# GaodeRender/triangle-splatting

Measured on AMD Instinct MI355X. Metric: fwd+bwd Mpixels/sec @ 1M triangles, 1920x1080; achieved HBM GB/s, higher is better.
Workload: dtype f32

## Files before the change

### triangle-splatting_amd/csrc/api.hip

```cpp
#pragma GCC visibility push(default)
#include "../../include/ts2d.h"
#ifdef TS2D_LAB
#include "ts2d_lab.h"
#endif
#pragma GCC visibility pop
#include "ts2d_api.h"
#include <atomic>
#include <chrono>
#include <cstdarg>
#include <cstdio>
#include <cstring>
#include <mutex>
#include <string>
#include <vector>

namespace
{
thread_local std::string g_err;

struct ProfRow { std::string name; double ms = 0; int64_t launches = 0; };
struct ProfPending { int row; hipEvent_t a, b; };
std::mutex g_prof_mu;
bool g_prof_on = false;
std::string g_prof_only;
std::vector<ProfRow> g_prof_rows;
std::vector<ProfPending> g_prof_pending;
std::vector<hipEvent_t> g_prof_free;

void prof_drain()
{
    for (auto &p : g_prof_pending)
    {
        float ms = 0;
        if (hipEventSynchronize(p.b) == hipSuccess && hipEventElapsedTime(&ms, p.a, p.b) == hipSuccess)
        {
            g_prof_rows[p.row].ms += ms;
            g_prof_rows[p.row].launches += 1;
        }
        g_prof_free.push_back(p.a);
        g_prof_free.push_back(p.b);
    }
    g_prof_pending.clear();
}

#ifdef TS2D_LAB
bool g_lab_all_quadrants = false;
bool g_lab_kernel_cull = false;
#endif

bool block_masks_in_keys(const ts2d_camera *cam, uint32_t flags)
{
    const int gx = (cam->width + TS_TILE - 1) / TS_TILE, gy = (cam->height + TS_TILE - 1) / TS_TILE;
    return !(flags & TS2D_FLAG_3D) && (int64_t)gx * gy <= TS_BLOCKMASK_MAX_TILES;
}

int validate(const ts2d_camera *cam, const ts2d_geometry *geom, uint32_t flags)
{
    if (!cam || !geom) return ts_fail(TS2D_ERR_INVALID, "null camera/geometry");
    if (cam->width <= 0 || cam->height <= 0) return ts_fail(TS2D_ERR_INVALID, "image size must be positive");
    if (cam->width > 65535 * TS_TILE || cam->height > 65535 * TS_TILE) return ts_fail(TS2D_ERR_INVALID, "image too large");
    if (geom->P < 0) return ts_fail(TS2D_ERR_INVALID, "P must be >= 0");
    if (geom->P > (int)TS_ID_MASK) return ts_fail(TS2D_ERR_CAPACITY, "more than 2^28 - 1 triangles: the instance values keep four bits for the quadrant mask");
    if (geom->C > TS2D_MAX_CHANNELS)
        return ts_fail(TS2D_ERR_INVALID, "feature's num_channels can't be larger than MAX_CHANNELS");
    if (geom->C < 1) return ts_fail(TS2D_ERR_INVALID, "need at least one colour channel");
    if (geom->gamma < 0.0f) return ts_fail(TS2D_ERR_INVALID, "gamma must be larger than 0");
    if (flags & TS2D_FLAG_USE_SHS)
    {
        if (geom->C != 3) return ts_fail(TS2D_ERR_INVALID, "SH mode renders 3 channels");
        if (geom->sh_degree < 0 || geom->sh_degree > 3) return ts_fail(TS2D_ERR_INVALID, "sh_degree must be in 0..3");
        if ((geom->sh_degree + 1) * (geom->sh_degree + 1) > geom->M)
            return ts_fail(TS2D_ERR_INVALID, "shs holds fewer coefficients than sh_degree needs");
        if (geom->P > 0 && !geom->shs) return ts_fail(TS2D_ERR_INVALID, "shs is null");
    }
    else if (geom->P > 0 && !geom->feature) return ts_fail(TS2D_ERR_INVALID, "feature is null");
    if (geom->P > 0 && (!geom->vertex || !geom->opacity)) return ts_fail(TS2D_ERR_INVALID, "vertex/opacity is null");
    if (!cam->viewmatrix || !cam->projmatrix || !cam->campos || !geom->background)
        return ts_fail(TS2D_ERR_INVALID, "camera matrices / background are null");
    return TS2D_OK;
}

PreprocessArgs make_pre(const ts2d_camera *cam, const ts2d_geometry *geom, uint32_t flags)
{
    PreprocessArgs a;
    a.W = cam->width; a.H = cam->height; a.P = geom->P; a.D = geom->sh_degree; a.M = geom->M; a.C = geom->C;
    a.grid_x = (cam->width + TS_TILE - 1) / TS_TILE; a.grid_y = (cam->height + TS_TILE - 1) / TS_TILE;
    a.rich_info = flags & TS2D_FLAG_RICH_INFO; a.use_shs = flags & TS2D_FLAG_USE_SHS;
    a.back_culling = flags & TS2D_FLAG_BACK_CULLING;
    a.tan_fovx = cam->tan_fovx; a.tan_fovy = cam->tan_fovy;
    a.viewmatrix = cam->viewmatrix; a.projmatrix = cam->projmatrix; a.campos = cam->campos;
    a.vertex = geom->vertex; a.shs = geom->shs; a.feature = geom->feature; a.opacity = geom->opacity;
    return a;
}

RenderArgs make_render(const ts2d_camera *cam, const ts2d_geometry *geom, uint32_t flags)
{
    RenderArgs r;
    r.W = cam->width; r.H = cam->height; r.C = geom->C;
    r.grid_x = (cam->width + TS_TILE - 1) / TS_TILE; r.grid_y = (cam->height + TS_TILE - 1) / TS_TILE;
    r.gamma = geom->gamma; r.background_depth = geom->background_depth;
    r.background_depth_dev = geom->background_depth_dev;
    r.background = geom->background;
    r.rich_info = flags & TS2D_FLAG_RICH_INFO;
    r.block_masks = block_masks_in_keys(cam, flags);
#ifdef TS2D_LAB
    if (g_lab_kernel_cull) r.block_masks = false;
#endif
    return r;
}

inline void cpu_relax()
{
#if defined(__x86_64__) || defined(__i386__)
    __builtin_ia32_pause();
#elif defined(__aarch64__)
    asm volatile("yield" ::: "memory");
#endif
}

struct CapacityHint { int dev, variant, W, H; unsigned long long key; double per_triangle; unsigned long long stamp; };
thread_local unsigned long long t_hint_key = 0;
std::atomic<unsigned long long> g_speculative_overflows{0};
std::mutex g_hint_mu;
std::vector<CapacityHint> g_hints;
unsigned long long g_hint_clock = 0;

void record_instance_count(int variant, int W, int H, int P, unsigned long long n)
{
    int dev = 0;
    if (P <= 0 || hipGetDevice(&dev) != hipSuccess) return;
    const double per = (double)n / (double)P;
    std::lock_guard<std::mutex> lk(g_hint_mu);
    CapacityHint *slot = nullptr;
    for (auto &h : g_hints)
        if (h.dev == dev && h.variant == variant && h.W == W && h.H == H && h.key == t_hint_key) slot = &h;
    if (!slot)
    {
        if (g_hints.size() < 32) { g_hints.push_back({dev, variant, W, H, t_hint_key, 0.0, 0}); slot = &g_hints.back(); }
        else
// ... 526 lines not shown
        if (dst_bytes < (size_t)N * 8) return ts_fail(TS2D_ERR_CAPACITY, "dst too small");
        std::vector<uint32_t> tile((size_t)N), vals((size_t)N), depth((size_t)P);
        if (N > 0)
        {
            TS_HIP(hipMemcpyAsync(tile.data(), b.tile, (size_t)N * 4, hipMemcpyDeviceToHost, s));
            TS_HIP(hipMemcpyAsync(vals.data(), b.vals, (size_t)N * 4, hipMemcpyDeviceToHost, s));
            TS_HIP(hipMemcpyAsync(depth.data(), g.depth, (size_t)P * 4, hipMemcpyDeviceToHost, s));
            TS_HIP(hipStreamSynchronize(s));
        }
        uint64_t *o = (uint64_t *)dst;
        const uint32_t keymask = ts_tile_keymask(gx * gy);
        for (int64_t i = 0; i < N; i++) o[i] = ((uint64_t)(tile[i] & keymask) << 32) | depth[vals[i] & TS_ID_MASK];
        return TS2D_OK;
    }
    case 11: src = b.vals; bytes = (size_t)N * 4; break;
    case 12: src = im.ranges; bytes = (size_t)gx * gy * 8; break;
    case 13: src = im.n_contrib; bytes = (size_t)W * H * 4; break;
    case 14: src = im.final_T; bytes = (size_t)W * H * 4; break;
    case 15: src = b.k[(b.passes & 1) ^ 1]; bytes = (size_t)N * 4; break;
    case 16: src = b.v[(b.passes & 1) ^ 1]; bytes = (size_t)N * 4; break;
    case 17:
    {
        uint32_t top_const = 0;
        if (P > 0)
        {
            TS_HIP(hipMemcpyAsync(&top_const, g.top_const, 4, hipMemcpyDeviceToHost, s));
            TS_HIP(hipStreamSynchronize(s));
        }
        src = top_const ? g.sv[0] : g.sv[1];
        bytes = (size_t)P * 4;
        break;
    }
    case 18: src = g.rec; bytes = (size_t)P * TS_REC_FLOATS * 4; break;
    default: return ts_fail(TS2D_ERR_INVALID, "unknown field %d", field);
    }
    if (dst_bytes < bytes) return ts_fail(TS2D_ERR_CAPACITY, "dst too small");
    if (bytes)
    {
        TS_HIP(hipMemcpyAsync(dst, src, bytes, hipMemcpyDeviceToHost, s));
        TS_HIP(hipStreamSynchronize(s));
    }
    return TS2D_OK;
}

void ts2d_lab_force_ticket_passes(int on) { ts_force_ticket_passes(on != 0); }
void ts2d_lab_force_all_quadrants(int on) { g_lab_all_quadrants = on != 0; }
void ts2d_lab_force_kernel_cull(int on) { g_lab_kernel_cull = on != 0; }
void ts2d_lab_force_depth_pass4(int on) { ts_force_depth_pass4(on != 0); }
void ts2d_lab_depth_split(int mode, int bucket_cap) { ts_lab_depth_split(mode, bucket_cap); }
#endif

void ts2d_profile_enable(int on)
{
    std::lock_guard<std::mutex> lk(g_prof_mu);
    g_prof_on = on != 0;
}
void ts2d_profile_only(const char *name)
{
    std::lock_guard<std::mutex> lk(g_prof_mu);
    g_prof_only = name ? name : "";
}
void ts2d_profile_reset(void)
{
    std::lock_guard<std::mutex> lk(g_prof_mu);
    prof_drain();
    g_prof_rows.clear();
}
int ts2d_profile_read(int32_t index, char *name, size_t name_bytes, double *total_ms, int64_t *launches)
{
    std::lock_guard<std::mutex> lk(g_prof_mu);
    prof_drain();
    if (index < 0 || (size_t)index >= g_prof_rows.size()) return TS2D_ERR_INVALID;
    const ProfRow &r = g_prof_rows[index];
    if (name && name_bytes) { strncpy(name, r.name.c_str(), name_bytes - 1); name[name_bytes - 1] = 0; }
    if (total_ms) *total_ms = r.ms;
    if (launches) *launches = r.launches;
    return TS2D_OK;
}
}
```

### triangle-splatting_amd/csrc/render_group.hip

```cpp
#include "ts2d_common.h"
#include "ts2d_wave.h"
#include "ts2d_group.h"
#include "ts2d_support.h"

#ifndef TSG_FWD_WAVES
#define TSG_FWD_WAVES 7
#endif
#ifndef TSG_BWD_WAVES
#define TSG_BWD_WAVES 7
#endif
#ifndef TSG_FWD_CAP
#define TSG_FWD_CAP 64
#endif
#ifndef TSG_BWD_CAP
#define TSG_BWD_CAP 64
#endif
#ifndef TSG_TCAP
#define TSG_TCAP 960
#endif
#ifndef TSG_PART
#define TSG_PART 3
#endif
namespace
{
// ... 73 lines not shown
    BlockCull s;
    entry_geometry(s, r0.x, r0.y, r0.z, r0.w, r1.x, r1.y, OX, OY);
#pragma unroll
    for (int g = 0; g < 4; g++) s.ov[g] = (id_nibble >> (TS_ID_BITS + g)) & 1u;
    return s;
}

__device__ __forceinline__ void write_dummy_row(float *row, int lane)
{
    if (lane < ROW)
    {
        float v = 0.0f;
        if (lane == 0 || lane == 1 || lane == 3 || lane == 4) v = 1000.0f;
        if (lane == 2 || lane == 5) v = 1001.0f;
        if (lane == 6) v = 1.0f;
        if (lane == 18) v = __int_as_float(0x7fffffff);
        row[lane] = v;
    }
}

struct Bary { float p1x, p1y, p2x, p2y, p3x, p3y, a1, a2, a3, mn, ecc; };
__device__ __forceinline__ Bary barycentrics(const float4 &q0, const float4 &q1, float fx, float fy)
{
    Bary b;
    b.p1x = q0.x - fx; b.p1y = q0.y - fy; b.p2x = q0.z - fx; b.p2y = q0.w - fy; b.p3x = q1.x - fx; b.p3y = q1.y - fy;
    b.a1 = (b.p2x * b.p3y - b.p2y * b.p3x) * q1.z;
    b.a2 = (b.p3x * b.p1y - b.p3y * b.p1x) * q1.z;
    b.a3 = 1.0f - b.a1 - b.a2;
    b.mn = fminf(fminf(b.a1, b.a2), b.a3);
    b.ecc = fmaf(-3.0f, b.mn, 1.0f);
    return b;
}
#ifdef TS2D_STATS
__device__ unsigned long long g_stats_group[12];
#define TSG_STAT(i, v) stat_acc[i] += (unsigned long long)(v)
#else
#define TSG_STAT(i, v)
#endif

#if TSG_PART & 1
template <bool RICH, bool GAMMA1, bool CULL>
__global__ void __launch_bounds__(256, TSG_FWD_WAVES) render_fwd_group_kernel(RenderArgs a, const uint2 *__restrict__ ranges,
                                                                const uint32_t *__restrict__ point_list, const uint32_t *__restrict__ keys,
                                                                const float4 *__restrict__ rec,
                                                                float *__restrict__ final_T, uint32_t *__restrict__ n_contrib,
                                                                float *__restrict__ out_feature, float *__restrict__ out_depth,
                                                                float *__restrict__ out_normal, float *__restrict__ contrib_sum,
                                                                float *__restrict__ contrib_max)
{
    __shared__ __attribute__((aligned(16))) float cst_all[4][(NR + 1) * ROW];
    __shared__ __attribute__((aligned(16))) uint32_t list_all[4][4 * NR / 2];
    constexpr int TCAP = TSG_TCAP;
    __shared__ unsigned long long tsum[RICH ? TCAP : 1];
    __shared__ int tmax[RICH ? TCAP : 1];

    const int tile = tile_of_block(blockIdx.x, a.grid_x, a.grid_y);
    if (tile < 0) return;
    const int wave = threadIdx.x >> 6;
    const GroupPixel p = group_pixel(a, tile, wave);
    const int lane = p.lane;
    const float fx = (float)p.lx, fy = (float)p.ly, OX = (float)p.X0, OY = (float)p.Y0;
    const uint2 range = ranges[tile];
    const int len = (int)(range.y - range.x);
    if (RICH) tile_stats_clear<TCAP>(tsum, tmax, len);
    const float g2 = 2.0f * a.gamma;
    float *cst = cst_all[wave] + ROW;
    uint32_t *list = list_all[wave];
    write_dummy_row(cst - ROW, lane);
    const char *lds0 = (const char *)cst_all;
    const uint32_t row0 = table_row0(wave, ROW), dummy = row0 - ROW * 4;
    const int stat_step = window_stat_step(lane);
    FwdPixel P = fwd_pixel(p.inside, len);

#ifdef TS2D_STATS
    unsigned long long stat_acc[12] = {0, 0, 0, 0, 0, 1, 0, 0, 0, 0, 0, 0};
#endif
    uint32_t id = 0;
    int pos = 0, cursor = 0;
    for (;;)
    {
        const unsigned long long alive = ballot(!P.done);
        if (alive == 0) break;
        int nq = 0;
        stream_refill<false, TSG_FWD_CAP, !CULL>(id, pos, nq, point_list + range.x, cursor, len, CULL ? TS_ID_BITS + wave : 16 + 4 * wave, lane,
                                                 keys + range.x);
        if (nq == 0) break;
        const bool valid = lane < nq;
        const int ent = pos;
        const uint32_t tid = CULL ? id : id & TS_ID_MASK;
        float4 r0 = make_float4(0, 0, 0, 0), r1 = r0, r2 = r0, r3 = r0;
        gather_record<RICH>(rec, tid, valid, r0, r1, r2, r3);
        const BlockCull s = entry_blocks<GAMMA1, CULL>(r0, r1, id, g2, OX, OY);
        unsigned long long M[4];
        const unsigned long long any = fwd_block_masks(M, alive, valid, s.ov);
        TSG_STAT(0, __popcll(ballot(valid)));
        if (any == 0) continue;
        TSG_STAT(1, __popcll(M[0]) + __popcll(M[1]) + __popcll(M[2]) + __popcll(M[3]));
        TSG_STAT(6, 1);
        TSG_STAT(7, __popcll(any));
        const Compaction cp = compact_rows(any, lane);
        bool mine = in_pass(cp, false);
        if (mine) publish_row(cst + cp.r * ROW, s, tid, ent, r1, r2, r3);
        for (int h = 0;;)
        {
            const int steps = build_lists(list, M, pass_mask(cp, mine), row0, cp.r, ROW, dummy, lane);
            const u16a *mylist = (const u16a *)list + p.grp * NR;
            TSG_STAT(2, steps);
            TSG_STAT(3, (steps + 7) / 8);
            TSG_STAT(8, __popcll(list_conflicts(list, dummy, lane)));
            TSG_STAT(9, 1);
            TSG_STAT(10, h > 0 ? 1 : 0);

            for (int t0 = 0; t0 < steps; t0 += 8)
            {
                float c[8];
                const uint4 packed = *(const uint4 *)(mylist + t0);
#pragma unroll
                for (int st = 0; st < 8; st++)
                {
                    c[st] = 0.0f;
                    if (t0 + st < steps)
                    {
                        const float *row = window_row(lds0, packed, st);
                        const float4 q0 = *(const float4 *)(row), q1 = *(const float4 *)(row + 4);
                        const Bary b = barycentrics(q0, q1, fx, fy);
                        const float4 q2 = *(const float4 *)(row + 8);
                        float4 q3 = make_float4(0, 0, 0, 0);
                        float vd3 = 0.0f;
                        int jpos;
                        if (RICH)
                        {
                            q3 = *(const float4 *)(row + 12);
                            const float4 q4 = *(const float4 *)(row + 16);
                            vd3 = q4.x;
                            jpos = __float_as_int(q4.z);
                        }
                        else jpos = __float_as_int(row[18]);
                        const float pw = GAMMA1 ? b.ecc * b.ecc : pow_nonneg(b.ecc, g2);
                        const float alpha = fminf(0.99f, q1.w * __builtin_amdgcn_exp2f(pw * -0.7213475204444817f));
                        const bool hit = !P.done && ecc_in_range(b.ecc) && alpha >= 1.0f / 255.0f;
                        TSG_STAT(4, __popcll(ballot(hit)));
                        const float d = q3.z * b.a1 + q3.w * b.a2 + vd3 * b.a3;
                        const float contrib = fwd_blend<RICH>(P, hit, alpha, q2.x, q2.y, q2.z, q2.w, q3.x, q3.y, d, jpos);
                        if (RICH) c[st] = contrib;
                    }
                }
                if (RICH) window_stats<TCAP>(c, lane, stat_step, lds0, mylist, t0, 18, tsum, tmax, point_list + range.x, contrib_sum, contrib_max);
            }
            if (++h * NR >= cp.nact) break;
            mine = in_pass(cp, true);
            if (mine) republish_row<RICH>(cst + cp.r * ROW, point_list, rec, range.x + pos, ent, OX, OY);
        }
    }

#ifdef TS2D_STATS
    if (lane == 0)
        for (int i = 0; i < 12; i++) atomicAdd(&g_stats_group[i], stat_acc[i]);
#endif
    fwd_store_pixel<RICH>(a, p, P, final_T, n_contrib, out_feature, out_depth, out_normal);
    if (RICH) tile_stats_leave<TCAP>(tsum, tmax, len, point_list + range.x, contrib_sum, contrib_max);
}

#endif

#if TSG_PART & 2
template <bool RICH, bool GAMMA1, bool CULL>
__global__ void __launch_bounds__(64, TSG_BWD_WAVES) render_bwd_group_kernel(RenderArgs a, const uint2 *__restrict__ ranges,
                                                             const uint32_t *__restrict__ point_list, const uint32_t *__restrict__ keys,
                                                             const float4 *__restrict__ rec,
                                                             const float *__restrict__ final_T, const uint32_t *__restrict__ n_contrib,
                                                             const float *__restrict__ dL_dout_feature,
                                                             const float *__restrict__ dL_dout_depth,
                                                             const float *__restrict__ dL_dout_normal, float *__restrict__ grad_rec)
{
    __shared__ __attribute__((aligned(16))) float rows_all[(NR + 1) * BROW];
    __shared__ __attribute__((aligned(16))) uint32_t list[4 * NR / 2];

    int quad;
    const int tile = tile_of_quadrant_block(blockIdx.x, a.grid_x, a.grid_y, quad);
    if (tile < 0) return;
    const GroupPixel p = group_pixel(a, tile, quad);
    const int lane = p.lane, grp = p.grp, sub = p.sub;
    const float fx = (float)p.lx, fy = (float)p.ly, OX = (float)p.X0, OY = (float)p.Y0;
    const uint2 range = ranges[tile];
    const float g2 = 2.0f * a.gamma;
    float *rows = rows_all + BROW;
    write_dummy_row(rows - BROW, lane);
    char *lds0 = (char *)rows_all;
    const uint32_t row0 = table_row0(0, BROW), dummy = row0 - BROW * 4;
    const uint32_t accoff = ROW * 4 + 4 * sub;

    const BwdPixel P = bwd_pixel<RICH>(a, p, final_T, n_contrib, dL_dout_feature, dL_dout_depth, dL_dout_normal);
    float T = P.T, B = P.B;
    const int last = P.last;
    const float dpr = P.dpr, dpg = P.dpg, dpb = P.dpb, dnx = P.dnx, dny = P.dny, dnz = P.dnz, dd = P.dd;
    const int quarter = sub >> 2;
    const float kq0 = quarter == 0 ? dpr : (quarter == 1 ? dpg : (quarter == 2 ? dpb : dnx));
    const float kq1 = quarter == 0 ? dpb : (quarter == 1 ? dnx : (quarter == 2 ? dpr : dpg));
    const float kq2 = quarter == 0 ? dpg : (quarter == 1 ? dpr : (quarter == 2 ? dnx : dpb));
    const float kq3 = quarter == 0 ? dnx : (quarter == 1 ? dpb : (quarter == 2 ? dpg : dpr));
    const float kp4 = (sub & 8) ? dnz : dny, kp5 = (sub & 8) ? dny : dnz;
    const int rcol = (int)((0xF15ADC39E0486B27ull >> (4 * sub)) & 15ull);
    int glast[4];
    const int maxlast = block_lasts(last, glast);
    if (maxlast <= 0) return;

    uint32_t id = 0;
    int pos = 0, cursor = maxlast;
    for (;;)
    {
        int nq = 0;
        stream_refill<true, TSG_BWD_CAP, !CULL>(id, pos, nq, point_list + range.x, cursor, maxlast, CULL ? TS_ID_BITS + quad : 16 + 4 * quad, lane,
                                                keys + range.x);
        if (nq == 0) break;
        const bool valid = lane < nq;
        const int ent = pos;
        const uint32_t tid = CULL ? id : id & TS_ID_MASK;
        float4 r0 = make_float4(0, 0, 0, 0), r1 = r0, r2 = r0, r3 = r0;
        gather_record<RICH>(rec, tid, valid, r0, r1, r2, r3);
        const BlockCull s = entry_blocks<GAMMA1, CULL>(r0, r1, id, g2, OX, OY);
        unsigned long long M[4];
        const unsigned long long any = bwd_block_masks(M, valid, s.ov, pos, glast);
        if (any == 0) continue;
        const Compaction cp = compact_rows(any, lane);
        bool mine = in_pass(cp, false);
        if (mine) publish_row(rows + cp.r * BROW, s, tid, ent, r1, r2, r3);
        for (int h = (cp.nact - 1) / NR;;)
        {
            const unsigned long long mm = pass_mask(cp, mine);
            if (mine) zero_sums(rows + cp.r * BROW + ROW);
            const int steps = build_lists(list, M, mm, row0, cp.r, BROW, dummy, lane);
            const u16a *mylist = (const u16a *)list + grp * NR;
            const unsigned long long conflict = list_conflicts(list, dummy, lane);
            uint32_t ra_next = mylist[0];
            for (int t0 = 0; t0 < steps; t0++)
            {
                {
                    const uint32_t ra = ra_next;
                    ra_next = mylist[min(t0 + 1, NR - 1)];
                    const float *row = (const float *)(lds0 + ra);
                    float *acc = (float *)(lds0 + ra + accoff);
                    const bool shared_row = (conflict >> t0) & 1;
                    const float q0acc = *acc;
                    const float4 q0 = *(const float4 *)(row), q1 = *(const float4 *)(row + 4);
                    const Bary b = barycentrics(q0, q1, fx, fy);
                    const float4 q2 = *(const float4 *)(row + 8);
                    float4 q3 = make_float4(0, 0, 0, 0);
                    float vd3 = 0.0f;
                    int jpos;
                    if (RICH)
                    {
                        q3 = *(const float4 *)(row + 12);
                        const float4 q4 = *(const float4 *)(row + 16);
                        vd3 = q4.x;
                        jpos = __float_as_int(q4.z);
                    }
                    else jpos = __float_as_int(row[18]);
                    const float pw = GAMMA1 ? b.ecc * b.ecc : pow_nonneg(b.ecc, g2);
                    const float G = __builtin_amdgcn_exp2f(pw * -0.7213475204444817f);
                    const float opG = q1.w * G;
                    const float alpha = fminf(0.99f, opG);
                    const bool hit = (jpos < last) && ecc_in_range(b.ecc) && alpha >= 1.0f / 255.0f;
                    const float al = hit ? alpha : 0.0f;
                    const float oma = 1.0f - al;
                    T = T * __builtin_amdgcn_rcpf(oma);
                    const float contrib = al * T;
// ... 24 lines not shown
                    v[6] = e3 * b.p2y - e2 * b.p3y;
                    v[7] = e2 * b.p3x - e3 * b.p2x;
                    v[8] = e1 * b.p3y - e3 * b.p1y;
                    v[9] = e3 * b.p1x - e1 * b.p3x;
                    v[10] = e2 * b.p1y - e1 * b.p2y;
                    v[11] = e1 * b.p2x - e2 * b.p1x;
                    v[12] = hit ? dL_dalpha * G : 0.0f;
                    v[13] = w * b.a1; v[14] = w * b.a2; v[15] = w * b.a3;
                    const float red = row_reduce16c(v, 0xCCCCCCCCCCCCCCCCull, 0xAAAAAAAAAAAAAAAAull);
                    row_add(acc, q0acc, red, shared_row, grp);
                }
            }

            {
                const int n = __popcll(mm);
#pragma unroll 1
                for (int e0 = 0; e0 < n; e0 += 4)
                {
                    const int e = e0 + grp;
                    if (e < n)
                    {
                        const uint32_t eid = __float_as_uint(rows[e * BROW + 17]);
                        float val = rows[e * BROW + ROW + sub];
                        if (rcol < 6) val *= rows[e * BROW + 6];
                        if (RICH || rcol < 10) unsafeAtomicAdd(grad_rec + TS_GRAD_FLOATS * (size_t)eid + rcol, val);
                    }
                }
            }
            if (--h < 0) break;
            mine = in_pass(cp, true);
            if (mine) republish_row<RICH>(rows + cp.r * BROW, point_list, rec, range.x + pos, ent, OX, OY);
        }
    }
}
#endif
}

#define TS_BLEND2D_RG(KERNEL, R, G1, A, GRID, BLOCK, STREAM, ...)                                                                  \
    do                                                                                                                            \
    {                                                                                                                             \
        if ((A).block_masks) hipLaunchKernelGGL((KERNEL<R, G1, false>), dim3(GRID), dim3(BLOCK), 0, STREAM, __VA_ARGS__);          \
        else hipLaunchKernelGGL((KERNEL<R, G1, true>), dim3(GRID), dim3(BLOCK), 0, STREAM, __VA_ARGS__);                          \
    } while (0)
#define TS_LAUNCH_BLEND2D(KERNEL, A, GRID, BLOCK, STREAM, ...)                                                                    \
    do                                                                                                                            \
    {                                                                                                                             \
        const bool g1 = ((A).gamma == 1.0f);                                                                                      \
        if ((A).rich_info && g1) TS_BLEND2D_RG(KERNEL, true, true, A, GRID, BLOCK, STREAM, __VA_ARGS__);                          \
        else if ((A).rich_info) TS_BLEND2D_RG(KERNEL, true, false, A, GRID, BLOCK, STREAM, __VA_ARGS__);                          \
        else if (g1) TS_BLEND2D_RG(KERNEL, false, true, A, GRID, BLOCK, STREAM, __VA_ARGS__);                                     \
        else TS_BLEND2D_RG(KERNEL, false, false, A, GRID, BLOCK, STREAM, __VA_ARGS__);                                            \
    } while (0)

#if TSG_PART & 1
void ts_launch_render_fwd_group(const RenderArgs &a, const GeometryStateView &g, const BinningStateView &b, const ImageStateView &im,
                                float *out_feature, float *out_depth, float *out_normal, float *contrib_sum, float *contrib_max,
                                hipStream_t s)
{
    if (a.grid_x * a.grid_y == 0) return;
    TS_LAUNCH_BLEND2D(render_fwd_group_kernel, a, ts_tile_units(a.grid_x, a.grid_y), 256, s, a, im.ranges, b.vals, b.tile, g.rec, im.final_T, im.n_contrib,
                      out_feature, out_depth, out_normal, contrib_sum, contrib_max);
}

#endif

#if defined(TS2D_STATS) && (TSG_PART & 1)
extern "C" __attribute__((visibility("default"))) int ts2d_stats_read_group(unsigned long long *out, int reset)
{
    hipError_t e = hipMemcpyFromSymbol(out, HIP_SYMBOL(g_stats_group), sizeof(unsigned long long) * 12);
    if (e == hipSuccess && reset)
    {
        unsigned long long z[12] = {0};
        e = hipMemcpyToSymbol(HIP_SYMBOL(g_stats_group), z, sizeof(z));
    }
    return e == hipSuccess ? 0 : 2;
}
#endif

#if TSG_PART & 2
void ts_launch_render_bwd_group(const RenderArgs &a, const GeometryStateView &g, const BinningStateView &b, const ImageStateView &im,
                                const float *dL_dout_feature, const float *dL_dout_depth, const float *dL_dout_normal, float *grad_rec,
                                hipStream_t s)
{
    if (a.grid_x * a.grid_y == 0) return;
    TS_LAUNCH_BLEND2D(render_bwd_group_kernel, a, ts_quadrant_units(a.grid_x, a.grid_y), 64, s, a, im.ranges, b.vals, b.tile, g.rec, im.final_T, im.n_contrib,
                      dL_dout_feature, dL_dout_depth, dL_dout_normal, grad_rec);
}
#endif
```

### triangle-splatting_amd/csrc/ts2d_common.h

```cpp
#pragma once
#include <hip/hip_runtime.h>
#include <stddef.h>
#include <stdint.h>

#define TS_TILE 16
#define TS_ALIGN 256

#define TS_REC_FLOATS 16

#define TS_ID_BITS 28
#define TS_ID_MASK 0x0FFFFFFFu
#define TS_GRAD_FLOATS 16

#ifndef TS_RS_CHUNK
#define TS_RS_CHUNK 4096
#endif
#define TS_RS_CHUNK_MID 2048
#define TS_RS_CHUNK_SMALL 1024
#define TS_RS_SMALL_BELOW 2500000
static inline int ts_instance_chunk(size_t n) { return n <= (size_t)TS_RS_SMALL_BELOW ? TS_RS_CHUNK_SMALL : TS_RS_CHUNK; }
static inline int ts_depth_chunk(size_t n) { return n <= (size_t)TS_RS_SMALL_BELOW ? TS_RS_CHUNK_SMALL : TS_RS_CHUNK_MID; }
#define TS_RS_BINS 256
#define TS_RS_TICKET_EXTRA 8
struct RadixScratchView
// ... 173 lines not shown
struct QuadMaskArgs
{
    int variant;
    float g2;
    float tan_fovx, tan_fovy;
    int W, H;
    float inv_W, inv_H;
    int blocks;
};
void ts_launch_zero_words(uint32_t *p, size_t n, hipStream_t s);
void ts_launch_emit_keys(int P, int grid_x, int ntiles, const GeometryStateView &g, const BinningStateView &b, const ImageStateView &im,
                         float *contrib_sum, float *contrib_max, int64_t capacity, int32_t *status, const QuadMaskArgs &qm, hipStream_t s);
const unsigned long long *ts_instance_count_dev(const GeometryStateView &g, int P);
void ts_sort_pairs(const BinningStateView &b, int64_t N, const unsigned long long *n_dev, int ntiles, hipStream_t s);
void ts_launch_tile_ranges(int64_t N, const unsigned long long *n_dev, int ntiles, const BinningStateView &b, const ImageStateView &im, hipStream_t s);
size_t ts_quantile_scratch_bytes();
void ts_quantile_threshold(const uint32_t *keys, size_t n, float q, void *scratch, float *thr, hipStream_t s);
void ts_quantile_passes(const uint32_t *keys, size_t n, float q, void *scratch, int first_pass, hipStream_t s);
size_t ts_quantile_state_words();
size_t ts_radix_scratch_bytes(size_t n);
int ts_radix_sort_pairs(uint32_t *const k[2], uint32_t *const v[2], size_t n, int end_bit, void *scratch, hipStream_t s, bool force_tickets = false);
void ts_force_ticket_passes(bool on);
void ts_force_depth_pass4(bool on);
void ts_lab_depth_split(int mode, int bucket_cap);

struct RenderArgs
{
    int W, H, C, grid_x, grid_y;
    float gamma, background_depth;
    const float *background;
    const float *background_depth_dev;
    bool rich_info;
    bool block_masks;
};
void ts_launch_render_fwd_group(const RenderArgs &a, const GeometryStateView &g, const BinningStateView &b,
                                const ImageStateView &im, float *out_feature, float *out_depth, float *out_normal,
                                float *contrib_sum, float *contrib_max, hipStream_t s);
void ts_launch_render_bwd_group(const RenderArgs &a, const GeometryStateView &g, const BinningStateView &b,
                                const ImageStateView &im, const float *dL_dout_feature, const float *dL_dout_depth,
                                const float *dL_dout_normal, float *grad_rec, hipStream_t s);
void ts_launch_preprocess_bwd(const PreprocessArgs &a, const int32_t *radii, const GeometryStateView &g,
                              const float *grad_rec, float *dL_dvertex, float *dL_dcenter2D, float *dL_dshs,
                              float *dL_dfeature, float *dL_dopacity, hipStream_t s);

void ts_launch_preprocess3d_fwd(const PreprocessArgs &a, int32_t *radii, const GeometryStateView &g, hipStream_t s);
void ts_launch_preprocess3d_bwd(const PreprocessArgs &a, const int32_t *radii, const GeometryStateView &g,
                                const float *grad_rec, float *dL_dvertex, float *dL_dcenter2D, float *dL_dshs,
                                float *dL_dfeature, float *dL_dopacity, hipStream_t s);

void ts_launch_render3d_fwd_group(const RenderArgs &a, float tan_fovx, float tan_fovy, const GeometryStateView &g,
                                  const BinningStateView &b, const ImageStateView &im, float *out_feature, float *out_depth,
                                  float *out_normal, float *contrib_sum, float *contrib_max, hipStream_t s);
void ts_launch_render3d_bwd_group(const RenderArgs &a, float tan_fovx, float tan_fovy, const GeometryStateView &g,
                                  const BinningStateView &b, const ImageStateView &im, const float *dL_dout_feature,
                                  const float *dL_dout_depth, const float *dL_dout_normal, float *grad_rec, hipStream_t s);

struct MeshArgs
{
    int W, H, V, F, grid_x, grid_y;
    float tan_fovx, tan_fovy, znear;
    const float *viewmatrix;
    const float *vertices;
    const int32_t *faces;
};
void ts_launch_mesh_preprocess(const MeshArgs &a, const GeometryStateView &g, hipStream_t s);
void ts_launch_mesh_resolve(const MeshArgs &a, const GeometryStateView &g, const BinningStateView &b, const ImageStateView &im,
// ... 70 lines not shown
```

### triangle-splatting_amd/csrc/ts2d_group.h

```cpp
#pragma once
#include "ts2d_common.h"
#include "ts2d_wave.h"

namespace
{
constexpr int NR = 32;
typedef unsigned short __attribute__((may_alias)) u16a;
constexpr int ROW = 20;

__device__ __forceinline__ unsigned long long ballot(bool p) { return __builtin_amdgcn_ballot_w64(p); }
__device__ __forceinline__ int lane_rank(unsigned long long m)
{
    return (int)__builtin_amdgcn_mbcnt_hi((uint32_t)(m >> 32), __builtin_amdgcn_mbcnt_lo((uint32_t)m, 0u));
}

__device__ __forceinline__ bool ecc_in_range(float ecc) { return __float_as_uint(ecc) <= 0x41200000u; }

template <bool DESC, int CAP = 64, bool NIB = false>
__device__ __forceinline__ void stream_refill(uint32_t &id, int &pos, int &n, const uint32_t *__restrict__ list, int &cursor, int end, int qbit, int lane,
                                              const uint32_t *__restrict__ keys = nullptr)
{
    while (n < CAP && (DESC ? cursor > 0 : cursor < end))
    {
        const int k = DESC ? cursor - 1 - lane : cursor + lane;
        const bool valid = DESC ? k >= 0 : k < end;
        uint32_t v = 0u, key = 0u;
        if (valid)
        {
            v = list[k];
            if (NIB) key = keys[k];
        }
        const uint32_t nib = NIB ? (key << (TS_ID_BITS - qbit)) & ~TS_ID_MASK : 0u;
        const bool want = NIB ? nib != 0u : valid && ((v >> qbit) & 1u);
        unsigned long long mt = ballot(want);
        int adv = 64;
        const int room = CAP - n;
        bool taken = want;
        if (__popcll(mt) > room)
        {
            taken = want && lane_rank(mt) < room;
// ... 235 lines not shown
    bool done;
    uint32_t last;
};
__device__ __forceinline__ FwdPixel fwd_pixel(bool inside, int len)
{
    return {1.0f, 0.0f, 0.0f, 0.0f, 0.0f, 0.0f, 0.0f, 0.0f, !inside, (uint32_t)len};
}
template <bool RICH>
__device__ __forceinline__ float fwd_blend(FwdPixel &P, bool hit, float alpha, float r, float g, float b, float nx, float ny, float nz, float d, int jpos)
{
    const float al = hit ? alpha : 0.0f;
    const float contrib = al * P.T;
    P.ar = fmaf(r, contrib, P.ar);
    P.ag = fmaf(g, contrib, P.ag);
    P.ab = fmaf(b, contrib, P.ab);
    if (RICH)
    {
        P.anx = fmaf(nx, contrib, P.anx);
        P.any_ = fmaf(ny, contrib, P.any_);
        P.anz = fmaf(nz, contrib, P.anz);
        P.ad = fmaf(d, contrib, P.ad);
    }
    P.T *= (1.0f - al);
    const bool sat = hit && P.T <= 0.0001f;
    P.last = sat ? (uint32_t)(jpos + 1) : P.last;
    P.done = P.done || sat;
    return contrib;
}
__device__ __forceinline__ const float *window_row(const char *lds0, const uint4 &packed, int st)
{
    const uint32_t word = st < 2 ? packed.x : (st < 4 ? packed.y : (st < 6 ? packed.z : packed.w));
    return (const float *)(lds0 + ((st & 1) ? (word >> 16) : (word & 0xFFFFu)));
}
template <int TCAP>
__device__ __forceinline__ void window_stats(const float (&c)[8], int lane, int stat_step, const char *lds0, const u16a *mylist, int t0, int slot,
                                             unsigned long long *tsum, int *tmax, const uint32_t *tile_list, float *contrib_sum, float *contrib_max)
{
    float sm, mx;
    row_reduce8_sum_max(c, 0xCCCCCCCCCCCCCCCCull, sm, mx);
    int k = 0;
    if ((lane & 1) == 0 && sm > 0.0f) k = __float_as_int(*(const float *)(lds0 + mylist[t0 + stat_step] + slot * 4));
    if ((lane & 1) == 0 && sm > 0.0f) tile_stats_add<TCAP>(tsum, tmax, k, sm, mx, tile_list, contrib_sum, contrib_max);
}
__device__ __forceinline__ int window_stat_step(int lane)
{
    return ((lane >> 3) & 1) | ((lane >> 1) & 2) | ((lane << 1) & 4);
}
template <int TCAP>
__device__ __forceinline__ void tile_stats_clear(unsigned long long *tsum, int *tmax, int len)
{
    for (int k = threadIdx.x; k < min(len, TCAP); k += 256) { tsum[k] = 0ull; tmax[k] = 0; }
    __syncthreads();
}
template <bool RICH>
__device__ __forceinline__ void fwd_store_pixel(const RenderArgs &a, const GroupPixel &p, const FwdPixel &P,
                                                float *__restrict__ final_T, uint32_t *__restrict__ n_contrib, float *__restrict__ out_feature,
                                                float *__restrict__ out_depth, float *__restrict__ out_normal)
{
    if (p.inside)
    {
        const size_t pix = (size_t)p.py * a.W + p.px, HW = (size_t)a.H * a.W;
        final_T[pix] = P.T;
        n_contrib[pix] = P.last;
        out_feature[pix] = P.ar + P.T * a.background[0];
        if (a.C > 1) out_feature[HW + pix] = P.ag + P.T * a.background[1];
        if (a.C > 2) out_feature[2 * HW + pix] = P.ab + P.T * a.background[2];
        if (RICH)
        {
            out_depth[pix] = P.ad + P.T * (a.background_depth_dev ? *a.background_depth_dev : a.background_depth);
            out_normal[pix] = P.anx;
            out_normal[HW + pix] = P.any_;
            out_normal[2 * HW + pix] = P.anz;
        }
    }
// ... 96 lines not shown
```

### triangle-splatting_amd/csrc/ts2d_lab.h

```cpp
#ifndef TS2D_LAB_H
#define TS2D_LAB_H

#include "../../include/ts2d.h"

#ifdef __cplusplus
extern "C" {
#endif

int ts2d_debug_read_state(const ts2d_state *state, int32_t P, int64_t num_rendered, int32_t width, int32_t height,
                          int32_t field, void *dst, size_t dst_bytes, void *stream);

int ts2d_test_sort_pairs(const uint32_t *keys_in, const uint32_t *vals_in, uint32_t *keys_out, uint32_t *vals_out, size_t n,
                         int32_t end_bit, int32_t which, void *stream);
int ts2d_test_inclusive_scan_rocprim(const uint32_t *in, uint32_t *out, size_t n, void *stream);

void ts2d_lab_force_ticket_passes(int on);
void ts2d_lab_force_depth_pass4(int on);
size_t ts2d_test_quantile_scratch_bytes(void);
int ts2d_test_quantile(const uint32_t *keys, size_t n, float q, void *scratch, float *out, void *stream);
void ts2d_lab_depth_split(int mode, int bucket_cap);
void ts2d_lab_force_all_quadrants(int on);
void ts2d_lab_force_kernel_cull(int on);

#ifdef __cplusplus
}
#endif
#endif
```

### triangle-splatting_amd/diff_triangle_rasterization_2D/_abi.py

```python
import ctypes as C

_vp = C.c_void_p


class _Camera(C.Structure):
    _fields_ = [("width", C.c_int32), ("height", C.c_int32), ("tan_fovx", C.c_float), ("tan_fovy", C.c_float),
                ("viewmatrix", _vp), ("projmatrix", _vp), ("campos", _vp)]


class _Geometry(C.Structure):
    _fields_ = [("P", C.c_int32), ("sh_degree", C.c_int32), ("M", C.c_int32), ("C", C.c_int32),
                ("gamma", C.c_float), ("scale_modifier", C.c_float), ("background_depth", C.c_float),
                ("background", _vp), ("vertex", _vp), ("shs", _vp), ("feature", _vp), ("opacity", _vp), ("background_depth_dev", _vp)]


class _ForwardOut(C.Structure):
    _fields_ = [("out_feature", _vp), ("depth", _vp), ("normal", _vp), ("contrib_sum", _vp), ("contrib_max", _vp)]


class _LossGrads(C.Structure):
    _fields_ = [("dL_dout_feature", _vp), ("dL_dout_depth", _vp), ("dL_dout_normal", _vp)]


class _BackwardOut(C.Structure):
# ... 93 lines not shown
    "tsm_split_vertex": (C.c_int, [C.c_int32, _vp, _vp, _vp, _vp, _vp]),
    "tsm_update_mask": (C.c_int, [C.c_int32, C.c_int32, _vp, _vp, _vp, C.c_float, C.c_float, _vp, _vp]),
    "tsm_clip": (C.c_int, [C.c_int32, C.c_int32, _vp, C.c_float, _vp, _vp, _vp, _vp]),
    "tsm_opacity_reset": (C.c_int, [C.c_int32, C.c_float, _vp, _vp, _vp, _vp]),
    "tsm_max_vertex_distance": (C.c_int, [C.c_int32, _vp, _vp, _vp, _vp]),
    "tsm_state_digest": (C.c_int, [C.c_int32, C.POINTER(_vp), C.POINTER(C.c_uint64), _vp, _vp]),
    "tso_adam_step": (C.c_int, [C.POINTER(_Slice), C.c_int32, C.c_double, C.c_double, C.c_double, _vp]),
    "tso_adam_step_sh_factored": (C.c_int, [C.POINTER(_ShFactoredStep), C.c_double, C.c_double, C.c_double, _vp]),
    "ts2d_mesh_geometry_state_bytes": (C.c_size_t, [C.c_int32]),
    "ts2d_mesh_bin": (C.c_int, [C.POINTER(_Camera), C.c_float, C.c_int32, _vp, C.c_int32, _vp, C.POINTER(_State), C.POINTER(C.c_int64), _vp]),
    "ts2d_mesh_render": (C.c_int, [C.POINTER(_Camera), C.c_int32, _vp, _vp, C.c_int64, C.POINTER(_State), _vp, _vp, _vp, _vp, _vp]),
    "ts2d_mesh_render_counted": (C.c_int, [C.POINTER(_Camera), C.c_int32, _vp, _vp, C.c_int64, C.POINTER(_State), _vp, _vp, _vp, _vp, _vp, _vp]),
    "ts2d_mesh_census_add": (C.c_int, [C.c_int32, C.c_int32, C.c_int32, _vp, _vp, _vp, _vp, _vp]),
    "ts2d_weld_workspace_bytes": (C.c_size_t, [C.c_int32, C.c_int32]),
    "ts2d_weld_labels": (C.c_int, [C.c_int32, _vp, C.c_float, _vp, _vp, C.c_size_t, _vp]),
    "ts2d_weld_labels_counted": (C.c_int, [C.c_int32, _vp, C.c_float, _vp, _vp, _vp, C.c_size_t, _vp]),
    "ts2d_weld_face_components": (C.c_int, [C.c_int32, C.c_int32, _vp, _vp, _vp, _vp, C.c_size_t, _vp]),
    "ts2d_weld_compact": (C.c_int, [C.c_int32, _vp, _vp, C.c_int32, _vp, _vp, _vp, _vp, C.c_size_t, _vp]),
    "ts2d_weld_remap_faces": (C.c_int, [C.c_int32, C.c_int32, _vp, _vp, _vp, _vp, _vp]),
    "ts2d_weld_edge_census": (C.c_int, [C.c_int32, C.c_int32, _vp, _vp, _vp, _vp, C.c_size_t, _vp]),
}

LAB_SIGNATURES = {
    "ts2d_debug_read_state": (C.c_int, [C.POINTER(_State), C.c_int32, C.c_int64, C.c_int32, C.c_int32, C.c_int32, _vp, C.c_size_t, _vp]),
    "ts2d_test_sort_pairs": (C.c_int, [_vp, _vp, _vp, _vp, C.c_size_t, C.c_int32, C.c_int32, _vp]),
    "ts2d_test_inclusive_scan_rocprim": (C.c_int, [_vp, _vp, C.c_size_t, _vp]),
    "ts2d_lab_force_ticket_passes": (None, [C.c_int]),
    "ts2d_lab_force_depth_pass4": (None, [C.c_int]),
    "ts2d_test_quantile_scratch_bytes": (C.c_size_t, []),
    "ts2d_test_quantile": (C.c_int, [_vp, C.c_size_t, C.c_float, _vp, _vp, _vp]),
    "ts2d_lab_depth_split": (None, [C.c_int, C.c_int]),
    "ts2d_lab_force_all_quadrants": (None, [C.c_int]),
    "ts2d_lab_force_kernel_cull": (None, [C.c_int]),
}

GEOM_SIGNATURES = {
    "tsg_last_error": (C.c_char_p, []),
    "tsg_cross_workspace_bytes": (C.c_size_t, [C.c_int32, C.c_int32]),
    "tsg_nearest_cross": (C.c_int, [C.c_int32, _vp, C.c_int32, _vp, _vp, _vp, _vp, _vp, C.c_size_t, _vp]),
    "tsg_sample_workspace_bytes": (C.c_size_t, [C.c_int32]),
    "tsg_face_areas": (C.c_int, [C.c_int32, C.c_int32, _vp, _vp, _vp, _vp, _vp]),
    "tsg_sample_surface": (C.c_int, [C.c_int32, C.c_int32, _vp, _vp, _vp, C.c_int32, C.c_uint64, _vp, _vp, _vp, C.c_size_t, _vp]),
}


BVH_SIGNATURES = {
    "tsb_last_error": (C.c_char_p, []),
    "tsb_bvh_bytes": (C.c_size_t, [C.c_int32]),
    "tsb_build_workspace_bytes": (C.c_size_t, [C.c_int32]),
    "tsb_build": (C.c_int, [C.c_int32, C.c_int32, _vp, _vp, _vp, _vp, C.c_size_t, _vp, C.c_size_t, _vp]),
    "tsb_closest_workspace_bytes": (C.c_size_t, [C.c_int32]),
    "tsb_closest": (C.c_int, [C.c_int32, _vp, C.c_int32, C.c_int32, _vp, _vp, _vp, C.c_size_t, _vp, _vp, _vp, _vp, _vp, C.c_size_t, _vp]),
}


RAY_SIGNATURES = {
    "tsr_last_error": (C.c_char_p, []),
    "tsr_cast_workspace_bytes": (C.c_size_t, [C.c_int32]),
    "tsr_cast": (C.c_int, [C.c_int32, _vp, _vp, _vp, C.c_double, C.c_double, C.c_int32, C.c_int32, _vp, C.c_size_t, _vp, _vp, _vp, _vp, _vp, _vp,
                           C.c_size_t, _vp]),
}


VOLUME_SIGNATURES = {
    "tsv_last_error": (C.c_char_p, []),
    "tsv_integrate": (C.c_int, [C.c_int32, C.c_int32, C.c_int32, C.c_float, C.c_float, C.c_float, C.c_float, C.c_float, _vp, C.c_float, C.c_float,
# ... 308 lines not shown
```

Before: 1354.

## Narrow per-instance block masks in forward so backward skips non-contributing blocks

```diff
diff --git a/triangle-splatting_amd/csrc/api.hip b/triangle-splatting_amd/csrc/api.hip
--- a/triangle-splatting_amd/csrc/api.hip
+++ b/triangle-splatting_amd/csrc/api.hip
@@ -46,6 +46,7 @@
 #ifdef TS2D_LAB
 bool g_lab_all_quadrants = false;
 bool g_lab_kernel_cull = false;
+bool g_lab_keep_masks = false;
 #endif
 
 bool block_masks_in_keys(const ts2d_camera *cam, uint32_t flags)
@@ -103,8 +104,10 @@
     r.background = geom->background;
     r.rich_info = flags & TS2D_FLAG_RICH_INFO;
     r.block_masks = block_masks_in_keys(cam, flags);
+    r.narrow_masks = r.block_masks;
 #ifdef TS2D_LAB
-    if (g_lab_kernel_cull) r.block_masks = false;
+    if (g_lab_kernel_cull) r.block_masks = r.narrow_masks = false;
+    if (g_lab_keep_masks) r.narrow_masks = false;
 #endif
     return r;
 }
@@ -697,6 +700,7 @@
         break;
     }
     case 18: src = g.rec; bytes = (size_t)P * TS_REC_FLOATS * 4; break;
+    case 19: src = b.tile; bytes = (size_t)N * 4; break;
     default: return ts_fail(TS2D_ERR_INVALID, "unknown field %d", field);
     }
     if (dst_bytes < bytes) return ts_fail(TS2D_ERR_CAPACITY, "dst too small");
@@ -711,6 +715,7 @@
 void ts2d_lab_force_ticket_passes(int on) { ts_force_ticket_passes(on != 0); }
 void ts2d_lab_force_all_quadrants(int on) { g_lab_all_quadrants = on != 0; }
 void ts2d_lab_force_kernel_cull(int on) { g_lab_kernel_cull = on != 0; }
+void ts2d_lab_keep_block_masks(int on) { g_lab_keep_masks = on != 0; }
 void ts2d_lab_force_depth_pass4(int on) { ts_force_depth_pass4(on != 0); }
 void ts2d_lab_depth_split(int mode, int bucket_cap) { ts_lab_depth_split(mode, bucket_cap); }
 #endif
diff --git a/triangle-splatting_amd/csrc/render_group.hip b/triangle-splatting_amd/csrc/render_group.hip
--- a/triangle-splatting_amd/csrc/render_group.hip
+++ b/triangle-splatting_amd/csrc/render_group.hip
@@ -129,16 +129,45 @@
     return b;
 }
 #ifdef TS2D_STATS
-__device__ unsigned long long g_stats_group[12];
+constexpr int TSG_NSTATS = 16;
+__device__ unsigned long long g_stats_group[TSG_NSTATS];
 #define TSG_STAT(i, v) stat_acc[i] += (unsigned long long)(v)
 #else
 #define TSG_STAT(i, v)
 #endif
 
 #if TSG_PART & 1
+__device__ __forceinline__ uint32_t group_or(uint32_t h)
+{
+    h |= (uint32_t)__builtin_amdgcn_update_dpp(0, (int)h, DPP_XOR1, 0xF, 0xF, false);
+    h |= (uint32_t)__builtin_amdgcn_update_dpp(0, (int)h, DPP_XOR2, 0xF, 0xF, false);
+    h |= (uint32_t)__builtin_amdgcn_update_dpp(0, (int)h, DPP_HALF_MIRROR, 0xF, 0xF, false);
+    h |= (uint32_t)__builtin_amdgcn_update_dpp(0, (int)h, DPP_MIRROR, 0xF, 0xF, false);
+    return h;
+}
+__device__ __forceinline__ uint32_t blended_blocks(uint32_t hist, int steps, const unsigned long long (&M)[4], unsigned long long mm, int lane)
+{
+    const uint32_t all = group_or(hist);
+    uint32_t blended = 0u;
+#pragma unroll
+    for (int g = 0; g < 4; g++)
+    {
+        const uint32_t seen = (uint32_t)__builtin_amdgcn_readlane((int)all, 16 * g);
+        const unsigned long long Mh = M[g] & mm;
+        if ((Mh >> lane) & 1) blended |= ((seen >> (steps - 1 - lane_rank(Mh))) & 1u) << g;
+    }
+    return blended;
+}
+__device__ __forceinline__ uint32_t narrow_key(uint32_t *key, uint32_t nib, uint32_t blended, int qbit)
+{
+    const uint32_t dead = nib & ~blended;
+    if (dead) atomicAnd(key, ~(dead << qbit));
+    return dead;
+}
+
 template <bool RICH, bool GAMMA1, bool CULL>
 __global__ void __launch_bounds__(256, TSG_FWD_WAVES) render_fwd_group_kernel(RenderArgs a, const uint2 *__restrict__ ranges,
-                                                                const uint32_t *__restrict__ point_list, const uint32_t *__restrict__ keys,
+                                                                const uint32_t *__restrict__ point_list, uint32_t *keys,
                                                                 const float4 *__restrict__ rec,
                                                                 float *__restrict__ final_T, uint32_t *__restrict__ n_contrib,
                                                                 float *__restrict__ out_feature, float *__restrict__ out_depth,
@@ -147,6 +176,7 @@
 {
     __shared__ __attribute__((aligned(16))) float cst_all[4][(NR + 1) * ROW];
     __shared__ __attribute__((aligned(16))) uint32_t list_all[4][4 * NR / 2];
+    constexpr bool HIST = !CULL && !RICH;
     constexpr int TCAP = TSG_TCAP;
     __shared__ unsigned long long tsum[RICH ? TCAP : 1];
     __shared__ int tmax[RICH ? TCAP : 1];
@@ -170,7 +200,7 @@
     FwdPixel P = fwd_pixel(p.inside, len);
 
 #ifdef TS2D_STATS
-    unsigned long long stat_acc[12] = {0, 0, 0, 0, 0, 1, 0, 0, 0, 0, 0, 0};
+    unsigned long long stat_acc[TSG_NSTATS] = {0, 0, 0, 0, 0, 1};
 #endif
     uint32_t id = 0;
     int pos = 0, cursor = 0;
@@ -202,6 +232,7 @@
         {
             const int steps = build_lists(list, M, pass_mask(cp, mine), row0, cp.r, ROW, dummy, lane);
             const u16a *mylist = (const u16a *)list + p.grp * NR;
+            uint32_t hist = 0u;
             TSG_STAT(2, steps);
             TSG_STAT(3, (steps + 7) / 8);
             TSG_STAT(8, __popcll(list_conflicts(list, dummy, lane)));
@@ -235,14 +266,25 @@
                         else jpos = __float_as_int(row[18]);
                         const float pw = GAMMA1 ? b.ecc * b.ecc : pow_nonneg(b.ecc, g2);
                         const float alpha = fminf(0.99f, q1.w * __builtin_amdgcn_exp2f(pw * -0.7213475204444817f));
+                        const float d = q3.z * b.a1 + q3.w * b.a2 + vd3 * b.a3;
                         const bool hit = !P.done && ecc_in_range(b.ecc) && alpha >= 1.0f / 255.0f;
                         TSG_STAT(4, __popcll(ballot(hit)));
-                        const float d = q3.z * b.a1 + q3.w * b.a2 + vd3 * b.a3;
+                        if (HIST) hist = hist + hist + (hit ? 1u : 0u);
                         const float contrib = fwd_blend<RICH>(P, hit, alpha, q2.x, q2.y, q2.z, q2.w, q3.x, q3.y, d, jpos);
                         if (RICH) c[st] = contrib;
                     }
                 }
-                if (RICH) window_stats<TCAP>(c, lane, stat_step, lds0, mylist, t0, 18, tsum, tmax, point_list + range.x, contrib_sum, contrib_max);
+                if (RICH)
+                    window_stats<TCAP, !CULL>(c, lane, stat_step, lds0, mylist, t0, 18, tsum, tmax, point_list + range.x, contrib_sum, contrib_max, 1u << p.grp,
+                                              a.narrow_masks, 19);
+            }
+            if (!CULL && a.narrow_masks)
+            {
+                const bool own = in_pass(cp, h > 0);
+                const uint32_t blended = RICH ? (own ? *(const u32a *)(cst + cp.r * ROW + 19) : 0u) : blended_blocks(hist, steps, M, pass_mask(cp, own), lane);
+                [[maybe_unused]] const uint32_t dead = own ? narrow_key(keys + range.x + ent, id >> TS_ID_BITS, blended, 16 + 4 * wave) : 0u;
+                TSG_STAT(11, __popcll(ballot(dead & 1u)) + __popcll(ballot(dead & 2u)) + __popcll(ballot(dead & 4u)) + __popcll(ballot(dead & 8u)));
+                TSG_STAT(12, __popcll(ballot(dead != 0u && dead == (id >> TS_ID_BITS))));
             }
             if (++h * NR >= cp.nact) break;
             mine = in_pass(cp, true);
@@ -252,7 +294,7 @@
 
 #ifdef TS2D_STATS
     if (lane == 0)
-        for (int i = 0; i < 12; i++) atomicAdd(&g_stats_group[i], stat_acc[i]);
+        for (int i = 0; i < TSG_NSTATS; i++) atomicAdd(&g_stats_group[i], stat_acc[i]);
 #endif
     fwd_store_pixel<RICH>(a, p, P, final_T, n_contrib, out_feature, out_depth, out_normal);
     if (RICH) tile_stats_leave<TCAP>(tsum, tmax, len, point_list + range.x, contrib_sum, contrib_max);
@@ -301,6 +343,9 @@
     int glast[4];
     const int maxlast = block_lasts(last, glast);
     if (maxlast <= 0) return;
+#ifdef TS2D_STATS
+    unsigned long long stat_acc[TSG_NSTATS] = {0, 0, 0, 0, 0, 1};
+#endif
 
     uint32_t id = 0;
     int pos = 0, cursor = maxlast;
@@ -319,6 +364,8 @@
         unsigned long long M[4];
         const unsigned long long any = bwd_block_masks(M, valid, s.ov, pos, glast);
         if (any == 0) continue;
+        TSG_STAT(1, __popcll(M[0]) + __popcll(M[1]) + __popcll(M[2]) + __popcll(M[3]));
+        TSG_STAT(7, __popcll(any));
         const Compaction cp = compact_rows(any, lane);
         bool mine = in_pass(cp, false);
         if (mine) publish_row(rows + cp.r * BROW, s, tid, ent, r1, r2, r3);
@@ -329,6 +376,7 @@
             const int steps = build_lists(list, M, mm, row0, cp.r, BROW, dummy, lane);
             const u16a *mylist = (const u16a *)list + grp * NR;
             const unsigned long long conflict = list_conflicts(list, dummy, lane);
+            TSG_STAT(2, steps);
             uint32_t ra_next = mylist[0];
             for (int t0 = 0; t0 < steps; t0++)
             {
@@ -419,6 +467,10 @@
             if (mine) republish_row<RICH>(rows + cp.r * BROW, point_list, rec, range.x + pos, ent, OX, OY);
         }
     }
+#ifdef TS2D_STATS
+    if (lane == 0)
+        for (int i = 0; i < TSG_NSTATS; i++) atomicAdd(&g_stats_group[i], stat_acc[i]);
+#endif
 }
 #endif
 }
@@ -451,17 +503,23 @@
 
 #endif
 
-#if defined(TS2D_STATS) && (TSG_PART & 1)
-extern "C" __attribute__((visibility("default"))) int ts2d_stats_read_group(unsigned long long *out, int reset)
-{
-    hipError_t e = hipMemcpyFromSymbol(out, HIP_SYMBOL(g_stats_group), sizeof(unsigned long long) * 12);
+#ifdef TS2D_STATS
+static int stats_read(unsigned long long *out, int n, int reset)
+{
+    hipError_t e = hipMemcpyFromSymbol(out, HIP_SYMBOL(g_stats_group), sizeof(unsigned long long) * n);
     if (e == hipSuccess && reset)
     {
-        unsigned long long z[12] = {0};
+        unsigned long long z[TSG_NSTATS] = {0};
         e = hipMemcpyToSymbol(HIP_SYMBOL(g_stats_group), z, sizeof(z));
     }
     return e == hipSuccess ? 0 : 2;
 }
+#if TSG_PART & 1
+extern "C" __attribute__((visibility("default"))) int ts2d_stats_read_group(unsigned long long *out, int reset) { return stats_read(out, 12, reset); }
+extern "C" __attribute__((visibility("default"))) int ts2d_stats_read_group_fwd(unsigned long long *out, int reset) { return stats_read(out, TSG_NSTATS, reset); }
+#else
+extern "C" __attribute__((visibility("default"))) int ts2d_stats_read_group_bwd(unsigned long long *out, int reset) { return stats_read(out, TSG_NSTATS, reset); }
+#endif
 #endif
 
 #if TSG_PART & 2
diff --git a/triangle-splatting_amd/csrc/ts2d_common.h b/triangle-splatting_amd/csrc/ts2d_common.h
--- a/triangle-splatting_amd/csrc/ts2d_common.h
+++ b/triangle-splatting_amd/csrc/ts2d_common.h
@@ -229,6 +229,7 @@
     const float *background_depth_dev;
     bool rich_info;
     bool block_masks;
+    bool narrow_masks;
 };
 void ts_launch_render_fwd_group(const RenderArgs &a, const GeometryStateView &g, const BinningStateView &b,
                                 const ImageStateView &im, float *out_feature, float *out_depth, float *out_normal,
diff --git a/triangle-splatting_amd/csrc/ts2d_group.h b/triangle-splatting_amd/csrc/ts2d_group.h
--- a/triangle-splatting_amd/csrc/ts2d_group.h
+++ b/triangle-splatting_amd/csrc/ts2d_group.h
@@ -6,6 +6,7 @@
 {
 constexpr int NR = 32;
 typedef unsigned short __attribute__((may_alias)) u16a;
+typedef uint32_t __attribute__((may_alias)) u32a;
 constexpr int ROW = 20;
 
 __device__ __forceinline__ unsigned long long ballot(bool p) { return __builtin_amdgcn_ballot_w64(p); }
@@ -307,14 +308,20 @@
     const uint32_t word = st < 2 ? packed.x : (st < 4 ? packed.y : (st < 6 ? packed.z : packed.w));
     return (const float *)(lds0 + ((st & 1) ? (word >> 16) : (word & 0xFFFFu)));
 }
-template <int TCAP>
+template <int TCAP, bool MARK = false>
 __device__ __forceinline__ void window_stats(const float (&c)[8], int lane, int stat_step, const char *lds0, const u16a *mylist, int t0, int slot,
-                                             unsigned long long *tsum, int *tmax, const uint32_t *tile_list, float *contrib_sum, float *contrib_max)
+                                             unsigned long long *tsum, int *tmax, const uint32_t *tile_list, float *contrib_sum, float *contrib_max,
+                                             uint32_t grpbit = 0u, bool mark = false, int mark_slot = 0)
 {
     float sm, mx;
     row_reduce8_sum_max(c, 0xCCCCCCCCCCCCCCCCull, sm, mx);
     int k = 0;
-    if ((lane & 1) == 0 && sm > 0.0f) k = __float_as_int(*(const float *)(lds0 + mylist[t0 + stat_step] + slot * 4));
+    if ((lane & 1) == 0 && sm > 0.0f)
+    {
+        const char *row = lds0 + mylist[t0 + stat_step];
+        k = __float_as_int(*(const float *)(row + slot * 4));
+        if (MARK && mark) __hip_atomic_fetch_or((u32a *)(row + mark_slot * 4), grpbit, __ATOMIC_RELAXED, __HIP_MEMORY_SCOPE_WORKGROUP);
+    }
     if ((lane & 1) == 0 && sm > 0.0f) tile_stats_add<TCAP>(tsum, tmax, k, sm, mx, tile_list, contrib_sum, contrib_max);
 }
 __device__ __forceinline__ int window_stat_step(int lane)
diff --git a/triangle-splatting_amd/csrc/ts2d_lab.h b/triangle-splatting_amd/csrc/ts2d_lab.h
--- a/triangle-splatting_amd/csrc/ts2d_lab.h
+++ b/triangle-splatting_amd/csrc/ts2d_lab.h
@@ -21,6 +21,7 @@
 void ts2d_lab_depth_split(int mode, int bucket_cap);
 void ts2d_lab_force_all_quadrants(int on);
 void ts2d_lab_force_kernel_cull(int on);
+void ts2d_lab_keep_block_masks(int on);
 
 #ifdef __cplusplus
 }
diff --git a/triangle-splatting_amd/diff_triangle_rasterization_2D/_abi.py b/triangle-splatting_amd/diff_triangle_rasterization_2D/_abi.py
--- a/triangle-splatting_amd/diff_triangle_rasterization_2D/_abi.py
+++ b/triangle-splatting_amd/diff_triangle_rasterization_2D/_abi.py
@@ -149,6 +149,7 @@
     "ts2d_lab_depth_split": (None, [C.c_int, C.c_int]),
     "ts2d_lab_force_all_quadrants": (None, [C.c_int]),
     "ts2d_lab_force_kernel_cull": (None, [C.c_int]),
+    "ts2d_lab_keep_block_masks": (None, [C.c_int]),
 }
 
 GEOM_SIGNATURES = {
```

Result: faster. 1380 (median of 6 runs) (+1.9%).
